# kaiwenShen/Do-You-Really-Need-to-Pay-2-20-Hedge-Fund-Strategy-Replication-via-Machine-Learning

Hardware: AMD Instinct MI355X
Metric: seq/sec/node MTSS-WGAN-GP train (24x32 windows) at 1/2/4/8 GPUs; W-dist parity (higher is better)
Workload: dtype fp32; 1 GPU; global_batch=262144, batch_per_gpu=262144, seq_len=24, features=32, parallelism=dp1

## Files before the change

do-you-really-need-to-pay-2-20-hedge-fund-strategy-replication-via-machine-learning_amd/csrc/lstmf_grad.hip:

```cpp
#include "lstmf_dev.h"

#include <stdexcept>
#include <type_traits>

namespace hfrep {

constexpr int WF_R = 16, WF_LA = 272, WF_LD = 400;
template <int KX>
struct WFGeo {
  static constexpr int KR = KX + FH + 1;
  static constexpr int NI = (KR + 15) / 16;
  static_assert(NI <= 16 && 16 * 16 <= WF_LA, "wgrad i tiles");
  static constexpr int NX4 = WF_R * KX / 4, NH4 = WF_R * FH / 4, ND4 = WF_R * FG / 4;
  static constexpr int JX = (NX4 + 511) / 512, JH = (NH4 + 511) / 512, JD = (ND4 + 511) / 512;
};

template <int KX, int XR = KX>
__global__ void __launch_bounds__(512)
lstmf_wgrad_kernel(const float* __restrict__ X, const float* __restrict__ Hs, const float* __restrict__ D,
                   const float* __restrict__ Xd, const float* __restrict__ Hds, const float* __restrict__ Dd,
                   float* __restrict__ slab, int M, int Tn, int rows_per_wg) {
  using WG = WFGeo<KX>;
  constexpr int NI = WG::NI, KR = WG::KR;
  __shared__ __attribute__((aligned(16))) float As[2][WF_R * WF_LA];
  __shared__ __attribute__((aligned(16))) float Ds[2][WF_R * WF_LD];
  __shared__ __attribute__((aligned(16))) float trash4[4];
  const int tid = threadIdx.x, lane = tid & 63;
  const int w = __builtin_amdgcn_readfirstlane(tid >> 6);
  const int g = lane >> 4, c16 = lane & 15;
  const int mb = blockIdx.x * rows_per_wg, me = min(M, mb + rows_per_wg);
  for (int i = tid; i < 2 * WF_R * WF_LA; i += 512) (&As[0][0])[i] = 0.f;

  f32x4 acc[NI][3], accx[2];
#pragma unroll
  for (int it = 0; it < NI; ++it)
#pragma unroll
    for (int jj = 0; jj < 3; ++jj) acc[it][jj] = f32x4{0.f, 0.f, 0.f, 0.f};
  accx[0] = accx[1] = f32x4{0.f, 0.f, 0.f, 0.f};
  const int ie0 = min(2 * w, 15), ie1 = min(2 * w + 1, 15);

  f32x4 vx[WG::JX], vh[WG::JH], vd[WG::JD];
  for (int seg = 0; seg < (Xd ? 2 : 1); ++seg) {
    const float* Xs = seg ? Xd : X;
    const float* Hq = seg ? Hds : Hs;
    const float* Dq = seg ? Dd : D;
    const int hb = mb > 0 ? mb - 1 : 0, nr = me > mb ? me - mb : 0;
    const rsrc_t rx = make_rsrc(Xs + (size_t)mb * XR, nr * XR * 4);
    const rsrc_t rh = make_rsrc(Hq + (size_t)hb * FH, (nr ? me - hb : 0) * FH * 4);
    const rsrc_t rd = make_rsrc(Dq + (size_t)mb * FG, nr * FG * 4);
    auto load = [&](int m0) {
#pragma unroll
      for (int j = 0; j < WG::JX; ++j) {
        const int e = tid + 512 * j, r = e / (KX / 4), c = e - r * (KX / 4);
        const bool ok = e < WG::NX4 && m0 + r < me;
        vx[j] = ldx4<XR>(rx, ok ? ((m0 - mb + r) * XR + 4 * c) * 4 : kOOB, 0, 4 * c);
      }
#pragma unroll
      for (int j = 0; j < WG::JH; ++j) {
        const int e = tid + 512 * j, r = e / (FH / 4), c = e - r * (FH / 4);
        const int m = m0 + r;
        const bool ok = e < WG::NH4 && m < me && (m % Tn) != 0;
        vh[j] = __builtin_bit_cast(f32x4, __builtin_amdgcn_raw_buffer_load_b128(rh, ok ? ((m - 1 - hb) * FH + 4 * c) * 4 : kOOB, 0, 0));
      }
#pragma unroll
      for (int j = 0; j < WG::JD; ++j) {
        const int e = tid + 512 * j, r = e / (FG / 4), c = e - r * (FG / 4);
        const bool ok = e < WG::ND4 && m0 + r < me;
        vd[j] = __builtin_bit_cast(f32x4, __builtin_amdgcn_raw_buffer_load_b128(rd, ok ? ((m0 - mb + r) * FG + 4 * c) * 4 : kOOB, 0, 0));
      }
    };
    auto to_lds = [&](int buf) {
#pragma unroll
      for (int j = 0; j < WG::JX; ++j) {
        const int e = tid + 512 * j, r = e / (KX / 4), c = e - r * (KX / 4);
        *reinterpret_cast<f32x4*>(e < WG::NX4 ? &As[buf][r * WF_LA + 4 * c] : trash4) = vx[j];
      }
#pragma unroll
      for (int j = 0; j < WG::JH; ++j) {
        const int e = tid + 512 * j, r = e / (FH / 4), c = e - r * (FH / 4);
        *reinterpret_cast<f32x4*>(e < WG::NH4 ? &As[buf][r * WF_LA + KX + 4 * c] : trash4) = vh[j];
      }
#pragma unroll
      for (int j = 0; j < WG::JD; ++j) {
        const int e = tid + 512 * j, r = e / (FG / 4), c = e - r * (FG / 4);
        *reinterpret_cast<f32x4*>(e < WG::ND4 ? &Ds[buf][r * WF_LD + 4 * c] : trash4) = vd[j];
      }
    };
    __syncthreads();
    if (tid < 2 * WF_R) As[tid >> 4][(tid & 15) * WF_LA + KR - 1] = seg ? 0.f : 1.f;
    if (mb < me) {
      load(mb);
      to_lds(0);
    }
    __syncthreads();
    int buf = 0;
    for (int m0 = mb; m0 < me; m0 += WF_R) {
      const bool more = m0 + WF_R < me;
      if (more) load(m0 + WF_R);
      const float* A_ = As[buf];
      const float* D_ = Ds[buf];
#pragma unroll
      for (int ks = 0; ks < 4; ++ks) {
        const float* ar = A_ + (4 * ks + g) * WF_LA + c16;
        const float* dr = D_ + (4 * ks + g) * WF_LD + c16;
        float a[NI], b[3];
#pragma unroll
        for (int it = 0; it < NI; ++it) a[it] = ar[16 * it];
#pragma unroll
        for (int jj = 0; jj < 3; ++jj) b[jj] = dr[16 * (3 * w + jj)];
        const float bx = dr[16 * 24], ax0 = ar[16 * ie0], ax1 = ar[16 * ie1];
#pragma unroll
        for (int it = 0; it < NI; ++it)
#pragma unroll
          for (int jj = 0; jj < 3; ++jj) acc[it][jj] = mma4(a[it], b[jj], acc[it][jj]);
        accx[0] = mma4(ax0, bx, accx[0]);
        accx[1] = mma4(ax1, bx, accx[1]);
      }
      if (more) to_lds(buf ^ 1);
      buf ^= 1;
      __syncthreads();
    }
  }
  float* out = slab + (size_t)blockIdx.x * KR * FG;
#pragma unroll
  for (int it = 0; it < NI; ++it)
#pragma unroll
    for (int jj = 0; jj < 3; ++jj)
#pragma unroll
      for (int r = 0; r < 4; ++r) {
        const int i = 16 * it + 4 * g + r;
        if (i < KR) out[(size_t)i * FG + 16 * (3 * w + jj) + c16] = acc[it][jj][r];
      }
#pragma unroll
  for (int e = 0; e < 2; ++e) {
    const int it = 2 * w + e;
#pragma unroll
    for (int r = 0; r < 4; ++r) {
      const int i = 16 * it + 4 * g + r;
      if (it < NI && i < KR) out[(size_t)i * FG + 16 * 24 + c16] = accx[e][r];
    }
  }
}

constexpr int WS_CA = 208, WS_CD = 208;
constexpr int ws_row_bytes(int cols, bool cf) {
  const int dw = (cols + 1) / 2;
  return 4 * (cf ? dw + ((8 - dw % 64) + 64) % 64 : (dw + 3) / 4 * 4);
}
template <int CA, int CD>
struct WImg {
  static constexpr bool CF = 2 * 3 * 32 * (ws_row_bytes(CA, true) + ws_row_bytes(CD, true)) <= 160 * 1024;
  static constexpr int ROWA = ws_row_bytes(CA, CF), ROWD = ws_row_bytes(CD, CF);
  static constexpr int PLA = 32 * ROWA, PLD = 32 * ROWD;
  static constexpr int IMGD = 3 * PLA;
  static constexpr int BUF = 3 * PLA + 3 * PLD;
  static_assert(2 * BUF <= 160 * 1024, "wgrad split LDS");
};

template <int KX>
struct WSGeo {
  static constexpr int KR = KX + FH + 1;
  static constexpr int NI = (KR + 15) / 16;
  static constexpr int NI0 = (NI + 1) / 2;
  static constexpr int JX = (32 * KX / 4 + 511) / 512, JH = (32 * FH / 4 + 511) / 512;
  static constexpr int JD = (32 * 52 + 511) / 512;
  static_assert(KX % 4 == 0 && 16 * NI <= WS_CA, "wgrad split: K");
  using Img = WImg<16 * NI, WS_CD>;
};

__device__ __forceinline__ int tr_lane_off(int lane, int rowb) {
  return (4 * (lane >> 4) + ((lane & 15) >> 2)) * rowb + 8 * (lane & 3);
}
template <int ROWB>
__device__ __forceinline__ bf16x8 tr_frag(const lds_char* img, int lane_off, int c0) {
  const s16x4 a = __builtin_amdgcn_ds_read_tr16_b64_v4i16((lds_s16x4*)(img + lane_off + c0 * 2));
  const s16x4 b = __builtin_amdgcn_ds_read_tr16_b64_v4i16((lds_s16x4*)(img + lane_off + 16 * ROWB + c0 * 2));
  return bf16x8{a[0], a[1], a[2], a[3], b[0], b[1], b[2], b[3]};
}

template <int NP>
__device__ __forceinline__ void wg_block(int Z, int& z, int& jp) {
  if (Z % 8 == 0) {
    const unsigned slot = blockIdx.x >> 3;
    jp = slot % NP;
    z = (slot / NP) * 8 + (blockIdx.x & 7);
  } else {
    jp = blockIdx.x % NP;
    z = blockIdx.x / NP;
  }
}
template <int BYTES>
__device__ __forceinline__ void wg_zero_lds(lds_char* wsm, int tid) {
  for (int i = tid; i < BYTES / 16; i += 512) reinterpret_cast<__attribute__((address_space(3))) u32x4_t*>(wsm)[i] = u32x4_t{0, 0, 0, 0};
}
template <class GI, int KR>
__device__ __forceinline__ void wg_bias_col(lds_char* wsm, int t, int seg) {
  if (t < 64) {
    const int buf = t >> 5, r = t & 31;
    *reinterpret_cast<__attribute__((address_space(3))) uint16_t*>(wsm + buf * GI::BUF + r * GI::ROWA + (KR - 1) * 2) =
        seg ? 0 : 0x3f80;
  }
}
struct WgRsrc {
  rsrc_t x, h, d;
};
template <int XR>
__device__ __forceinline__ WgRsrc wg_rsrc(const float* X, const float* H, const float* D, int mb, int nr, int jbase, int ncol) {
  return {make_rsrc(X + (size_t)mb * XR, nr * XR * 4), make_rsrc(H + ((ptrdiff_t)mb - 1) * FH, (nr ? nr + 1 : 0) * FH * 4),
          make_rsrc(D + (size_t)mb * FG + jbase, nr ? ((nr - 1) * FG + ncol) * 4 : 0)};
}
__device__ __forceinline__ int wg_tm0(int mb, int r, int Tn) { return (mb + r) % Tn; }
__device__ __forceinline__ void wg_tm_next(int& tm, int step32, int Tn) {
  tm += step32;
  if (tm >= Tn) tm -= Tn;
}
struct WgSlot {
  int r, c4;
  bool ok;
};
template <int PER>
__device__ __forceinline__ WgSlot wg_slot(int e) {
  const int r = e / PER;
  return {r, e - r * PER, e < 32 * PER};
}
template <int PER>
__device__ __forceinline__ WgSlot wg_slot(int e, int nc4) {
  WgSlot s = wg_slot<PER>(e);
  s.ok = s.ok && s.c4 < nc4;
  return s;
}
template <int RS>
__device__ __forceinline__ int wg_goff(const WgSlot& s) { return s.ok ? (s.r * RS + 4 * s.c4) * 4 : kOOB; }
template <int ROWB, int IMG>
__device__ __forceinline__ int wg_loff(const WgSlot& s) { return s.ok ? s.r * ROWB + IMG + 8 * s.c4 : -1; }
template <class GI>
__device__ __forceinline__ void wg_tr_bases(int lane, int (&tro_a)[2], int (&tro_d)[2]) {
#pragma unroll
  for (int b = 0; b < 2; ++b) {
    tro_a[b] = tr_lane_off(lane, GI::ROWA) + b * GI::BUF;
    tro_d[b] = tr_lane_off(lane, GI::ROWD) + b * GI::BUF + GI::IMGD;
    asm volatile("" : "+v"(tro_a[b]), "+v"(tro_d[b]));
  }
}
template <int KR>
__device__ __forceinline__ void wg_store_tile(float* out, const f32x4& acc, int it, int jt, int jbase, int ncol, int lane) {
  const int g = lane >> 4, col = 16 * jt + (lane & 15);
#pragma unroll
  for (int r = 0; r < 4; ++r) {
    const int i = 16 * it + 4 * g + r;
    if (i < KR && col < ncol) out[(size_t)i * FG + jbase + col] = acc[r];
  }
}

template <class GI, int NIV, int NJV, int NA, int NB>
__device__ __forceinline__ void ws_chunk(f32x4 (&acc)[NA][NB], const lds_char* A_, const lds_char* D_, int tro_a,
                                         int tro_d, int i0, int j0) {
  bf16x8 bfr[NJV][3];
#pragma unroll
  for (int jj = 0; jj < NJV; ++jj)
#pragma unroll
    for (int q = 0; q < 3; ++q) bfr[jj][q] = tr_frag<GI::ROWD>(D_ + q * GI::PLD, tro_d, 16 * (j0 + jj));
#pragma unroll
  for (int ii = 0; ii < NIV; ++ii) {
    __builtin_amdgcn_sched_barrier(0);
    bf16x8 a3[3];
#pragma unroll
    for (int q = 0; q < 3; ++q) a3[q] = tr_frag<GI::ROWA>(A_ + q * GI::PLA, tro_a, 16 * (i0 + ii));
#pragma unroll
    for (int j2 = 0; j2 < NJV; j2 += 2) {
      f32x4 t[2];
#pragma unroll
      for (int jj = j2; jj < j2 + 2 && jj < NJV; ++jj) t[jj - j2] = mma_split6(a3, bfr[jj], f32x4{0.f, 0.f, 0.f, 0.f});
#pragma unroll
      for (int jj = j2; jj < j2 + 2 && jj < NJV; ++jj) acc[ii][jj] += t[jj - j2];
    }
  }
}

template <int KX, int XR = KX>
__global__ void __launch_bounds__(512, 1)
lstmf_wgrad_split_kernel(const float* __restrict__ X, const float* __restrict__ Hs, const float* __restrict__ D,
                         const float* __restrict__ Xd, const float* __restrict__ Hds, const float* __restrict__ Dd,
                         float* __restrict__ slab, int M, int Tn, int rows_per_z, int Z) {
  constexpr int XRB = 4 * XR, HRB = 4 * FH, DRB = 4 * FG;
  using G = WSGeo<KX>;
  using GI = typename G::Img;
  constexpr int NI = G::NI, NI0 = G::NI0, JX = G::JX, JH = G::JH, JD = G::JD;
  extern __shared__ __attribute__((aligned(16))) char wsm_[];
  lds_char* wsm = (lds_char*)wsm_;
  const int tid = threadIdx.x, lane = tid & 63;
  const int w = __builtin_amdgcn_readfirstlane(tid >> 6);
  int z, jh;
  wg_block<2>(Z, z, jh);
  const int mb = z * rows_per_z, me = min(M, mb + rows_per_z);
  const int jbase = WS_CD * jh, nd4 = jh ? 48 : 52;

  const int ig = w >> 2, jg = ig ? 3 - (w & 3) : (w & 3);
  const int i0 = ig ? NI0 : 0, ni = ig ? NI - NI0 : NI0;
  const int j0 = jg == 0 ? 0 : 1 + 3 * jg, nj = jg == 0 ? 4 : 3;

  wg_zero_lds<2 * GI::BUF>(wsm, tid);
  __syncthreads();

  f32x4 acc[NI0][4];
#pragma unroll
  for (int a = 0; a < NI0; ++a)
#pragma unroll
    for (int b = 0; b < 4; ++b) acc[a][b] = f32x4{0.f, 0.f, 0.f, 0.f};

  const int tro_a = tr_lane_off(lane, GI::ROWA);
  int tro_d = tr_lane_off(lane, GI::ROWD) + GI::IMGD;
  asm volatile("" : "+v"(tro_d));

  int gx[JX], lx[JX], gh[JH], lh[JH], rhr[JH], gd[JD], ld_[JD], rd_[JD];
#pragma unroll
  for (int j = 0; j < JX; ++j) {
    const int e = tid + 512 * j, r = e / (KX / 4), c4 = e - r * (KX / 4);
    const bool ok = e < 32 * KX / 4;
    gx[j] = ok ? (r * XR + 4 * c4) * 4 : kOOB;
    lx[j] = ok ? r * GI::ROWA + 8 * c4 : -1;
  }
#pragma unroll
  for (int j = 0; j < JH; ++j) {
    const int e = tid + 512 * j, r = e / (FH / 4), c4 = e - r * (FH / 4);
    const bool ok = e < 32 * FH / 4;
    gh[j] = ok ? (r * FH + 4 * c4) * 4 : kOOB;
    lh[j] = ok ? r * GI::ROWA + 2 * KX + 8 * c4 : -1;
    rhr[j] = ok ? r : 0;
  }
#pragma unroll
  for (int j = 0; j < JD; ++j) {
    const int e = tid + 512 * j, r = e / 52, c4 = e - r * 52;
    const bool ok = e < 32 * 52 && c4 < nd4;
    gd[j] = ok ? (r * FG + jbase + 4 * c4) * 4 : kOOB;
    ld_[j] = ok ? GI::IMGD + r * GI::ROWD + 8 * c4 : -1;
    rd_[j] = ok ? r : 0;
  }
  const int step32 = 32 % Tn;

  f32x4 vx[JX], vh[JH], vd[JD];
  for (int seg = 0; seg < (Xd ? 2 : 1); ++seg) {
    const char* Xs = reinterpret_cast<const char*>(seg ? Xd : X);
    const char* Hq = reinterpret_cast<const char*>(seg ? Hds : Hs);
    const char* Dq = reinterpret_cast<const char*>(seg ? Dd : D);
    const int nr = me > mb ? me - mb : 0;
    const rsrc_t rx = make_rsrc(Xs + (size_t)mb * XRB, nr * XRB);
    const rsrc_t rh = make_rsrc(Hq + ((ptrdiff_t)mb - 1) * HRB, (nr ? nr + 1 : 0) * HRB);
    const rsrc_t rd = make_rsrc(Dq + (size_t)mb * DRB, nr * DRB);
    int tm[JH];
#pragma unroll
    for (int j = 0; j < JH; ++j) tm[j] = wg_tm0(mb, rhr[j], Tn);
    auto load = [&](int m0) {
      const int lim = me - m0;
#pragma unroll
      for (int j = 0; j < JX; ++j) {
        vx[j] = ldx4<XR>(rx, (gx[j] >> 2) / XR < lim ? gx[j] : kOOB, (m0 - mb) * XRB, (gx[j] >> 2) % XR);
      }
#pragma unroll
      for (int j = 0; j < JH; ++j) {
        const int vo = rhr[j] < lim && tm[j] != 0 ? gh[j] : kOOB;
        vh[j] = ld4s(rh, vo, (m0 - mb) * HRB);
      }
#pragma unroll
      for (int j = 0; j < JD; ++j) {
        const int vo = rd_[j] < lim ? gd[j] : kOOB;
        vd[j] = ld4s(rd, vo, (m0 - mb) * DRB);
      }
#pragma unroll
      for (int j = 0; j < JH; ++j) {
        wg_tm_next(tm[j], step32, Tn);
      }
    };
    auto put = [&](lds_char* base, int lo, const f32x4& v) {
      if (lo >= 0) {
        uint32_t p[3][2];
        split3(v, p);
        const int pl = lo < GI::IMGD ? GI::PLA : GI::PLD;
#pragma unroll
        for (int q = 0; q < 3; ++q)
          *reinterpret_cast<__attribute__((address_space(3))) u32x2_t*>(base + lo + q * pl) = u32x2_t{p[q][0], p[q][1]};
      }
    };
    auto stage = [&](int buf) {
      lds_char* base = wsm + buf * GI::BUF;
#pragma unroll
      for (int j = 0; j < JX; ++j) put(base, lx[j], vx[j]);
#pragma unroll
      for (int j = 0; j < JH; ++j) put(base, lh[j], vh[j]);
#pragma unroll
      for (int j = 0; j < JD; ++j) put(base, ld_[j], vd[j]);
    };
    wg_bias_col<GI, G::KR>(wsm, tid, seg);
    const int nch = nr > 0 ? (nr + 31) / 32 : 0;
    if (nch > 0) {
      load(mb);
      stage(0);
    }
    __syncthreads();
    for (int c = 0; c < nch; ++c) {
      const bool more = c + 1 < nch;
      if (more) load(mb + 32 * (c + 1));
      const lds_char* A_ = wsm + (c & 1) * GI::BUF;
      const lds_char* D_ = A_;
      switch (ni * 8 + nj) {
        case NI0 * 8 + 4: ws_chunk<GI, NI0, 4>(acc, A_, D_, tro_a, tro_d, i0, j0); break;
        case NI0 * 8 + 3: ws_chunk<GI, NI0, 3>(acc, A_, D_, tro_a, tro_d, i0, j0); break;
        case (NI - NI0) * 8 + 4: ws_chunk<GI, NI - NI0, 4>(acc, A_, D_, tro_a, tro_d, i0, j0); break;
        default: ws_chunk<GI, NI - NI0, 3>(acc, A_, D_, tro_a, tro_d, i0, j0); break;
      }
      if (more) stage((c + 1) & 1);
      __syncthreads();
    }
    __syncthreads();
  }
  float* out = slab + (size_t)z * G::KR * FG;
  const int g = lane >> 4, c16 = lane & 15;
#pragma unroll
  for (int ii = 0; ii < NI0; ++ii)
#pragma unroll
    for (int jj = 0; jj < 4; ++jj)
      if (ii < ni && jj < nj) {
        const int col = jbase + 16 * (j0 + jj) + c16;
#pragma unroll
        for (int r = 0; r < 4; ++r) {
          const int i = 16 * (i0 + ii) + 4 * g + r;
          if (i < G::KR && col < FG) out[(size_t)i * FG + col] = acc[ii][jj][r];
        }
      }
}

constexpr int WQ_CD = 100, WQ_NJ = 7, WQ_W = 8;
template <int KX>
struct WQGeo {
  static constexpr int KR = KX + FH + 1;
  static constexpr int NI = (KR + 15) / 16;
  static constexpr int NIG = (NI + 3) / 4;
  static constexpr int MAXT = NIG * 4;
  static constexpr int JX = (32 * KX / 4 + 511) / 512, JH = (32 * FH / 4 + 511) / 512;
  static constexpr int JD = (32 * WQ_CD / 4 + 511) / 512;
  static constexpr int NS = JX + JH + JD;
  static_assert(KX % 4 == 0 && 16 * NI <= WS_CA && NI <= 16, "wgrad q4: K");
  static constexpr int ig(int w) { return w < 4 ? w : 3 - (w & 3); }
  static constexpr int i0(int g) { return g == 0 ? 0 : NIG + (g - 1) * ((NI - NIG) / 3) + ((g - 1) < (NI - NIG) % 3 ? g - 1 : (NI - NIG) % 3); }
  static constexpr int ni(int g) { return i0(g + 1 > 3 ? 3 : g + 1) - i0(g) + (g == 3 ? NI - i0(3) : 0); }
  static constexpr int j0(int w) { return w < 4 ? 0 : 4; }
  static constexpr int nj(int w) { return w < 4 ? 4 : 3; }
  using Img = WImg<16 * NI, 16 * WQ_NJ>;
};

template <int KX>
__global__ void __launch_bounds__(512, 1)
lstmf_wgrad_q4_kernel(const float* __restrict__ X, const float* __restrict__ Hs, const float* __restrict__ D,
                      const float* __restrict__ Xd, const float* __restrict__ Hds, const float* __restrict__ Dd,
                      float* __restrict__ slab, int M, int Tn, int rows_per_z, int Z) {
  constexpr int XRB = 4 * KX, HRB = 4 * FH, DRB = 4 * FG;
  using G = WQGeo<KX>;
  using GI = typename G::Img;
  constexpr int JX = G::JX, JH = G::JH, NS = G::NS, MAXT = G::MAXT;
  extern __shared__ __attribute__((aligned(16))) char wsm_[];
  lds_char* wsm = (lds_char*)wsm_;
  const int tid = threadIdx.x, lane = tid & 63;
  const int w = __builtin_amdgcn_readfirstlane(tid >> 6);
  int z, jq;
  wg_block<4>(Z, z, jq);
  const int mb = z * rows_per_z, me = min(M, mb + rows_per_z);
  const int jbase = WQ_CD * jq;

  wg_zero_lds<2 * GI::BUF>(wsm, tid);
  __syncthreads();

  f32x4 acc[MAXT];
#pragma unroll
  for (int a = 0; a < MAXT; ++a) acc[a] = f32x4{0.f, 0.f, 0.f, 0.f};

  int tro_a[2], tro_d[2];
#pragma unroll
  for (int b = 0; b < 2; ++b) {
    tro_a[b] = tr_lane_off(lane, GI::ROWA) + b * GI::BUF;
    tro_d[b] = tr_lane_off(lane, GI::ROWD) + b * GI::BUF + GI::IMGD;
    asm volatile("" : "+v"(tro_a[b]), "+v"(tro_d[b]));
  }
  const int step32 = 32 % Tn;

  auto slot_rc = [&](int s, int& r, int& c4, bool& ok) {
    WgSlot sl;
    if (s < JX) sl = wg_slot<KX / 4>(tid + 512 * s);
    else if (s < JX + JH) sl = wg_slot<FH / 4>(tid + 512 * (s - JX));
    else sl = wg_slot<WQ_CD / 4>(tid + 512 * (s - JX - JH));
    r = sl.r; c4 = sl.c4; ok = sl.ok;
    if (!ok) r = c4 = 0;
  };

  f32x4 v[NS];
  for (int seg = 0; seg < (Xd ? 2 : 1); ++seg) {
    const char* Xs = reinterpret_cast<const char*>(seg ? Xd : X);
    const char* Hq = reinterpret_cast<const char*>(seg ? Hds : Hs);
    const char* Dq = reinterpret_cast<const char*>(seg ? Dd : D);
    const int nr = me > mb ? me - mb : 0;
    const rsrc_t rx = make_rsrc(Xs + (size_t)mb * XRB, nr * XRB);
    const rsrc_t rh = make_rsrc(Hq + ((ptrdiff_t)mb - 1) * HRB, (nr ? nr + 1 : 0) * HRB);
    const rsrc_t rd = make_rsrc(Dq + (size_t)mb * DRB + jbase * 4, nr ? (nr - 1) * DRB + WQ_CD * 4 : 0);
    int tm[JH];
#pragma unroll
    for (int j = 0; j < JH; ++j) {
      int r, c4;
      bool ok;
      slot_rc(JX + j, r, c4, ok);
      tm[j] = wg_tm0(mb, r, Tn);
    }
    auto load_slot = [&](int s, int m0) {
      int r, c4;
      bool ok;
      slot_rc(s, r, c4, ok);
      ok = ok && r < me - m0;
      if (s < JX) {
        v[s] = ld4s(rx, ok ? (r * KX + 4 * c4) * 4 : kOOB, (m0 - mb) * XRB);
      } else if (s < JX + JH) {
        int& tmj = tm[s - JX];
        v[s] = ld4s(rh, ok && tmj != 0 ? (r * FH + 4 * c4) * 4 : kOOB, (m0 - mb) * HRB);
        tmj += step32;
        if (tmj >= Tn) tmj -= Tn;
      } else {
        v[s] = ld4s(rd, ok ? (r * FG + 4 * c4) * 4 : kOOB, (m0 - mb) * DRB);
      }
    };
    auto stage = [&](lds_char* base, int s) {
      int r, c4;
      bool ok;
      slot_rc(s, r, c4, ok);
      if (!ok) return;
      int lo, pl;
      if (s < JX) { lo = r * GI::ROWA + 8 * c4; pl = GI::PLA; }
      else if (s < JX + JH) { lo = r * GI::ROWA + 2 * KX + 8 * c4; pl = GI::PLA; }
      else { lo = GI::IMGD + r * GI::ROWD + 8 * c4; pl = GI::PLD; }
      uint32_t p[3][2];
      split3(v[s], p);
#pragma unroll
      for (int q = 0; q < 3; ++q)
        *reinterpret_cast<__attribute__((address_space(3))) u32x2_t*>(base + lo + q * pl) = u32x2_t{p[q][0], p[q][1]};
    };
    using I0 = std::integral_constant<int, 0>;
    using I1 = std::integral_constant<int, 1>;
    wg_bias_col<GI, G::KR>(wsm, tid, seg);
    const int nch = nr > 0 ? (nr + 31) / 32 : 0;
#pragma unroll
    for (int s = 0; s < NS; ++s) load_slot(s, mb);
#pragma unroll
    for (int s = 0; s < NS; ++s) stage(wsm, s);
#pragma unroll
    for (int s = 0; s < NS; ++s) load_slot(s, mb + 32);
    __syncthreads();
    auto chunk = [&](auto S_, int c) {
      constexpr int S = decltype(S_)::value;
      const lds_char* A_ = wsm;
      const lds_char* D_ = wsm;
      lds_char* nxt = wsm + (S ^ 1) * GI::BUF;
      auto body = [&](auto WK) {
        constexpr int W = decltype(WK)::value;
        constexpr int IG = G::ig(W), I0 = G::i0(IG), NIW = G::ni(IG), J0 = G::j0(W), NJW = G::nj(W);
        constexpr int NJH = (NJW + 1) / 2;
        constexpr int SPI = (NS + NJH * NIW - 1) / (NJH * NIW);
        auto jpair = [&](auto JH_) {
          constexpr int jh = decltype(JH_)::value;
          bf16x8 bfr[2][3];
#pragma unroll
          for (int jj = 0; jj < 2; ++jj)
            if (2 * jh + jj < NJW) {
#pragma unroll
              for (int q = 0; q < 3; ++q) bfr[jj][q] = tr_frag<GI::ROWD>(D_ + q * GI::PLD, tro_d[S], 16 * (J0 + 2 * jh + jj));
            }
          constexpr bool PF = KX <= 36;
          bf16x8 af[2][3];
#pragma unroll
          for (int q = 0; q < 3; ++q) af[0][q] = tr_frag<GI::ROWA>(A_ + q * GI::PLA, tro_a[S], 16 * I0);
#pragma unroll
          for (int ii = 0; ii < NIW; ++ii) {
            __builtin_amdgcn_sched_barrier(0);
            if (PF && ii + 1 < NIW) {
#pragma unroll
              for (int q = 0; q < 3; ++q) af[(ii + 1) & 1][q] = tr_frag<GI::ROWA>(A_ + q * GI::PLA, tro_a[S], 16 * (I0 + ii + 1));
            } else if (!PF && ii > 0) {
#pragma unroll
              for (int q = 0; q < 3; ++q) af[ii & 1][q] = tr_frag<GI::ROWA>(A_ + q * GI::PLA, tro_a[S], 16 * (I0 + ii));
            }
            const bf16x8(&a3)[3] = af[ii & 1];
#pragma unroll
            for (int jj = 0; jj < 2; ++jj) {
              if (2 * jh + jj >= NJW) continue;
              acc[ii * 4 + 2 * jh + jj] += mma_split6(a3, bfr[jj], f32x4{0.f, 0.f, 0.f, 0.f});
            }
            const int it = jh * NIW + ii;
#pragma unroll
            for (int s = it * SPI; s < (it + 1) * SPI && s < NS; ++s) {
              stage(nxt, s);
              load_slot(s, mb + 32 * (c + 2));
            }
          }
        };
        jpair(std::integral_constant<int, 0>{});
        if constexpr (NJH > 1) jpair(std::integral_constant<int, 1>{});
      };
      switch (w) {
        case 0: body(std::integral_constant<int, 0>{}); break;
        case 1: body(std::integral_constant<int, 1>{}); break;
        case 2: body(std::integral_constant<int, 2>{}); break;
        case 3: body(std::integral_constant<int, 3>{}); break;
        case 4: body(std::integral_constant<int, 4>{}); break;
        case 5: body(std::integral_constant<int, 5>{}); break;
        case 6: body(std::integral_constant<int, 6>{}); break;
        default: body(std::integral_constant<int, 7>{}); break;
      }
      __syncthreads();
    };
    int c = 0;
    for (; c + 1 < nch; c += 2) {
      chunk(I0{}, c);
      chunk(I1{}, c + 1);
    }
    if (c < nch) chunk(I0{}, c);
    __syncthreads();
  }
  float* out = slab + (size_t)z * G::KR * FG;
  const int g = lane >> 4, c16 = lane & 15;
  const int igw = G::ig(w), i0w = G::i0(igw), niw = G::ni(igw), j0w = G::j0(w), njw = G::nj(w);
#pragma unroll
  for (int ii = 0; ii < G::NIG; ++ii)
#pragma unroll
    for (int jj = 0; jj < 4; ++jj) {
      const int col = 16 * (j0w + jj) + c16;
#pragma unroll
      for (int r = 0; r < 4; ++r) {
        const int i = 16 * (i0w + ii) + 4 * g + r;
        if (ii < niw && jj < njw && i < G::KR && col < WQ_CD)
          out[(size_t)i * FG + jbase + col] = acc[ii * 4 + jj][r];
      }
    }
}

#ifndef HFREP_WGRAD_ROLES_APF
#define HFREP_WGRAD_ROLES_APF 1
#endif
#ifndef HFREP_WGRAD_ROLES_PRIO
#define HFREP_WGRAD_ROLES_PRIO 0
#endif
template <int KX>
struct WRGeo {
  static constexpr bool QUAD = KX > 36;
  static constexpr int NP = QUAD ? 4 : 2;
  static constexpr int CDP = QUAD ? WQ_CD : WS_CD;
  static constexpr int NJ = (CDP + 15) / 16;
  static constexpr int KR = KX + FH + 1;
  static constexpr int NI = (KR + 15) / 16;
  static constexpr int NT = NI * NJ;
  static constexpr int ts(int w) { return w * (NT / 4) + (w < NT % 4 ? w : NT % 4); }
  static constexpr int MAXT = (NT + 3) / 4;
  static constexpr int ND4 = CDP / 4;
  static constexpr int JX = (32 * KX / 4 + 255) / 256, JH = (32 * FH / 4 + 255) / 256, JD = (32 * ND4 + 255) / 256;
  static constexpr int NS = JX + JH + JD;
  static_assert(KX % 4 == 0 && CDP % 4 == 0 && 16 * NI <= WS_CA && MAXT * 4 <= 120, "wgrad roles: K");
  using Img = WImg<16 * NI, 16 * NJ>;
};

template <int KX>
__global__ void __launch_bounds__(512, 1)
lstmf_wgrad_roles_kernel(const float* __restrict__ X, const float* __restrict__ Hs, const float* __restrict__ D,
                         const float* __restrict__ Xd, const float* __restrict__ Hds, const float* __restrict__ Dd,
                         float* __restrict__ slab, int M, int Tn, int rows_per_z, int Z) {
  using G = WRGeo<KX>;
  using GI = typename G::Img;
  constexpr int NI = G::NI, NP = G::NP, JX = G::JX, JH = G::JH, NS = G::NS;
  constexpr int XRB = 4 * KX, HRB = 4 * FH, DRB = 4 * FG;
  extern __shared__ __attribute__((aligned(16))) char wsm_[];
  lds_char* wsm = (lds_char*)wsm_;
  const int tid = threadIdx.x, lane = tid & 63;
  const int w = __builtin_amdgcn_readfirstlane(tid >> 6);
  int z, jp;
  wg_block<NP>(Z, z, jp);
  const int mb = z * rows_per_z, me = min(M, mb + rows_per_z);
  const int jbase = G::CDP * jp, ncol = min(G::CDP, FG - jbase);
  const int nr = me > mb ? me - mb : 0, nch = (nr + 31) / 32;
  const int nseg = Xd ? 2 : 1;

  wg_zero_lds<2 * GI::BUF>(wsm, tid);
  __syncthreads();

  using I0 = std::integral_constant<int, 0>;
  using I1 = std::integral_constant<int, 1>;
  if (w < 4) {
    auto role = [&](auto WK) {
      constexpr int W = decltype(WK)::value;
      constexpr int TS = G::ts(W), TE = G::ts(W + 1), JA = TS / NI, NJW = (TE - 1) / NI - JA + 1;
      f32x4 acc[TE - TS];
#pragma unroll
      for (int a = 0; a < TE - TS; ++a) acc[a] = f32x4{0.f, 0.f, 0.f, 0.f};
      int tro_a[2], tro_d[2];
      wg_tr_bases<GI>(lane, tro_a, tro_d);
      auto chunk = [&](auto S_) {
        constexpr int S = decltype(S_)::value;
        bf16x8 bfr[NJW][3];
#pragma unroll
        for (int jj = 0; jj < NJW; ++jj)
#pragma unroll
          for (int q = 0; q < 3; ++q) bfr[jj][q] = tr_frag<GI::ROWD>(wsm + q * GI::PLD, tro_d[S], 16 * (JA + jj));
        constexpr int PF = HFREP_WGRAD_ROLES_APF;
        bf16x8 af[PF + 1][3];
#pragma unroll
        for (int i = 0; i < PF; ++i)
#pragma unroll
          for (int q = 0; q < 3; ++q) af[i][q] = tr_frag<GI::ROWA>(wsm + q * GI::PLA, tro_a[S], 16 * i);
        f32x4 t[2];
        int pend = -1, par = 0;
#pragma unroll
        for (int ii = 0; ii < NI; ++ii) {
          __builtin_amdgcn_sched_barrier(0);
          if (ii + PF < NI) {
#pragma unroll
            for (int q = 0; q < 3; ++q) af[(ii + PF) % (PF + 1)][q] = tr_frag<GI::ROWA>(wsm + q * GI::PLA, tro_a[S], 16 * (ii + PF));
          }
          __builtin_amdgcn_sched_barrier(0);
          const bf16x8(&a3)[3] = af[ii % (PF + 1)];
#pragma unroll
          for (int jj = 0; jj < NJW; ++jj) {
            const int L = (JA + jj) * NI + ii;
            if (L < TS || L >= TE) continue;
            t[par] = mma_split6(a3, bfr[jj], f32x4{0.f, 0.f, 0.f, 0.f});
            __builtin_amdgcn_sched_barrier(0);
            if (pend >= 0) acc[pend] += t[par ^ 1];
            pend = L - TS;
            par ^= 1;
            __builtin_amdgcn_sched_barrier(0);
          }
        }
        acc[pend] += t[par ^ 1];
      };
#if HFREP_WGRAD_ROLES_PRIO
      __builtin_amdgcn_s_setprio(1);
#endif
      for (int seg = 0; seg < nseg; ++seg) {
        lds_barrier();
        int c = 0;
        for (; c + 1 < nch; c += 2) {
          chunk(I0{});
          lds_barrier();
          chunk(I1{});
          lds_barrier();
        }
        if (c < nch) {
          chunk(I0{});
          lds_barrier();
        }
      }
      float* out = slab + (size_t)z * G::KR * FG;
#pragma unroll
      for (int n = 0; n < TE - TS; ++n) wg_store_tile<G::KR>(out, acc[n], (TS + n) % NI, (TS + n) / NI, jbase, ncol, lane);
    };
    switch (w) {
      case 0: role(std::integral_constant<int, 0>{}); break;
      case 1: role(std::integral_constant<int, 1>{}); break;
      case 2: role(std::integral_constant<int, 2>{}); break;
      default: role(std::integral_constant<int, 3>{}); break;
    }
  } else {
    const int st = tid - 256;
    int gv[NS], lo[NS], rr[NS];
#pragma unroll
    for (int s = 0; s < NS; ++s) {
      WgSlot sl;
      if (s < JX) {
        sl = wg_slot<KX / 4>(st + 256 * s);
        gv[s] = wg_goff<KX>(sl);
        lo[s] = wg_loff<GI::ROWA, 0>(sl);
      } else if (s < JX + JH) {
        sl = wg_slot<FH / 4>(((st + 64) & 255) + 256 * (s - JX));
        gv[s] = wg_goff<FH>(sl);
        lo[s] = wg_loff<GI::ROWA, 2 * KX>(sl);
      } else {
        sl = wg_slot<G::ND4>(((st + 128) & 255) + 256 * (s - JX - JH), ncol / 4);
        gv[s] = wg_goff<FG>(sl);
        lo[s] = wg_loff<GI::ROWD, GI::IMGD>(sl);
      }
      rr[s] = sl.ok ? sl.r : 0;
    }
    const int step32 = 32 % Tn;
    f32x4 v[2][NS];
    for (int seg = 0; seg < nseg; ++seg) {
      const WgRsrc rs = wg_rsrc<KX>(seg ? Xd : X, seg ? Hds : Hs, seg ? Dd : D, mb, nr, jbase, ncol);
      int tm[JH];
#pragma unroll
      for (int j = 0; j < JH; ++j) tm[j] = wg_tm0(mb, rr[JX + j], Tn);
      auto load = [&](auto Q_, int m0) {
        constexpr int Q = decltype(Q_)::value;
        const int lim = me - m0;
#pragma unroll
        for (int s = 0; s < NS; ++s) {
          const bool in = rr[s] < lim;
          if (s < JX) {
            v[Q][s] = ld4s(rs.x, in ? gv[s] : kOOB, (m0 - mb) * XRB);
          } else if (s < JX + JH) {
            int& tmj = tm[s - JX];
            v[Q][s] = ld4s(rs.h, in && tmj != 0 ? gv[s] : kOOB, (m0 - mb) * HRB);
            wg_tm_next(tmj, step32, Tn);
          } else {
            v[Q][s] = ld4s(rs.d, in ? gv[s] : kOOB, (m0 - mb) * DRB);
          }
        }
      };
      auto stage = [&](auto Q_, int buf) {
        constexpr int Q = decltype(Q_)::value;
        lds_char* base = wsm + buf * GI::BUF;
#pragma unroll
        for (int s = 0; s < NS; ++s) {
          if (lo[s] >= 0) split3_store(v[Q][s], base + lo[s], s < JX + JH ? GI::PLA : GI::PLD);
        }
      };
      wg_bias_col<GI, G::KR>(wsm, st, seg);
      load(I0{}, mb);
      stage(I0{}, 0);
      load(I1{}, mb + 32);
      lds_barrier();
      int c = 0;
      for (; c + 1 < nch; c += 2) {
        load(I0{}, mb + 32 * (c + 2));
        stage(I1{}, 1);
        lds_barrier();
        load(I1{}, mb + 32 * (c + 3));
        stage(I0{}, 0);
        lds_barrier();
      }
      if (c < nch) {
        load(I0{}, mb + 32 * (c + 2));
        stage(I1{}, 1);
        lds_barrier();
      }
    }
  }
}

constexpr int DS4_RS = 432;
constexpr int DS4_PL = 16 * DS4_RS * 2;
constexpr int DS4_BUF = 3 * DS4_PL;
constexpr int DS4_SLOTS = (16 * 100 + 255) / 256;
constexpr int DS4_K0 = DS_KS - DS4_SLOTS;
constexpr int DS4_NS = 2;

template <int NT2>
__global__ void __launch_bounds__(256, 1)
lstmf_dgrad_s4_kernel(const float* __restrict__ D, const float* __restrict__ W, float* __restrict__ X, int M, int KO) {
  constexpr int DRB = 4 * FG;
  extern __shared__ __attribute__((aligned(16))) char dsm_[];
  lds_char* dsm = (lds_char*)dsm_;
  const int tid = threadIdx.x, lane = tid & 63;
  const int w = __builtin_amdgcn_readfirstlane(tid >> 6);
  const int g = lane >> 4, c16 = lane & 15;
  const int nch = (M + 15) / 16;
  bf16x8 bw[2][DS_KS][3];
#pragma unroll
  for (int e = 0; e < 2; ++e) {
    const int col = 16 * (2 * w + e) + c16;
#pragma unroll
    for (int ks = 0; ks < DS_KS; ++ks) {
      const int k0 = 32 * ks + 8 * g;
      f32x4 v0 = f32x4{0.f, 0.f, 0.f, 0.f}, v1 = v0;
      if (w < NT2 && col < KO && k0 < FG) {
        v0 = *reinterpret_cast<const f32x4*>(W + (size_t)col * FG + k0);
        v1 = *reinterpret_cast<const f32x4*>(W + (size_t)col * FG + k0 + 4);
      }
      uint32_t p0[3][2], p1[3][2];
      split3(v0, p0);
      split3(v1, p1);
#pragma unroll
      for (int q = 0; q < 3; ++q) {
        bw[e][ks][q] = __builtin_bit_cast(bf16x8, make_uint4(p0[q][0], p0[q][1], p1[q][0], p1[q][1]));
        if (e == 1) asm volatile("" : "+a"(bw[e][ks][q]));
      }
    }
  }
  f32x4 v[DS4_NS][DS4_SLOTS];
  auto load = [&](auto S_, int c) {
    constexpr int S = decltype(S_)::value;
    const int r0 = c * 16, nr = c < nch ? min(16, M - r0) : 0;
    const rsrc_t rd = make_rsrc(reinterpret_cast<const char*>(D) + (nr ? (size_t)r0 * DRB : 0), nr * DRB);
#pragma unroll
    for (int j = 0; j < DS4_SLOTS; ++j) {
      const int e = tid + 256 * j, r = e / 100, c4 = e - 100 * r;
      v[S][j] = ld4(rd, e < 1600 ? (r * FG + 4 * c4) * 4 : kOOB);
    }
  };
  auto stage = [&](auto S_, lds_char* buf, int j) {
    constexpr int S = decltype(S_)::value;
    const int e = tid + 256 * j, r = e / 100, c4 = e - 100 * r;
    if (e >= 1600) return;
    const int lo = (r * DS4_RS + 4 * c4) * 2;
    split3_store(v[S][j], buf + lo, DS4_PL);
  };
  for (int i = tid; i < 2 * 3 * 16 * 2; i += 256) {
    const int h = i & 1, b = i / 96, q = (i / 32) % 3, r = (i / 2) % 16;
    *reinterpret_cast<__attribute__((address_space(3))) u32x4_t*>(dsm + b * DS4_BUF + q * DS4_PL +
                                                                  (r * DS4_RS + FG + 8 * h) * 2) = u32x4_t{0, 0, 0, 0};
  }
  using I0 = std::integral_constant<int, 0>;
  using I1 = std::integral_constant<int, 1>;
  const int cs = gridDim.x;
  load(I0{}, blockIdx.x);
#pragma unroll
  for (int j = 0; j < DS4_SLOTS; ++j) stage(I0{}, dsm, j);
  load(I1{}, blockIdx.x + cs);
  __syncthreads();
  const int ao = (c16 * DS4_RS + 8 * g) * 2;
  auto chunk = [&](auto S_, int cc, int P) {
    constexpr int S = decltype(S_)::value, SN = (S + 1) % DS4_NS;
    load(S_, cc + DS4_NS * cs);
    const lds_char* A_ = dsm + P * DS4_BUF;
    lds_char* nxt = dsm + (P ^ 1) * DS4_BUF;
    f32x4 acc[2] = {f32x4{0.f, 0.f, 0.f, 0.f}, f32x4{0.f, 0.f, 0.f, 0.f}};
    bf16x8 af[2][3];
#pragma unroll
    for (int q = 0; q < 3; ++q) af[0][q] = *reinterpret_cast<const __attribute__((address_space(3))) bf16x8*>(A_ + q * DS4_PL + ao);
#pragma unroll
    for (int ks = 0; ks < DS_KS; ++ks) {
      __builtin_amdgcn_sched_barrier(0);
      if (ks + 1 < DS_KS) {
#pragma unroll
        for (int q = 0; q < 3; ++q)
          af[(ks + 1) & 1][q] = *reinterpret_cast<const __attribute__((address_space(3))) bf16x8*>(A_ + q * DS4_PL + ao + 64 * (ks + 1));
      }
      const bf16x8(&a)[3] = af[ks & 1];
#pragma unroll
      for (int e = 0; e < 2; ++e) acc[e] = mma_split6(a, bw[e][ks], acc[e]);
      if (ks >= DS4_K0) {
        stage(std::integral_constant<int, SN>{}, nxt, ks - DS4_K0);
#pragma unroll
        for (int i = 0; i < 12; ++i) {
          __builtin_amdgcn_sched_group_barrier(0x008, 1, 0);
          __builtin_amdgcn_sched_group_barrier(0x002, 2, 0);
        }
      }
    }
    const int nr = min(16, M - 16 * cc);
    const rsrc_t rx = make_rsrc(X + (size_t)16 * cc * KO, nr * KO * 4);
#pragma unroll
    for (int e = 0; e < 2; ++e) {
      const int col = 16 * (2 * w + e) + c16;
      const bool ok = w < NT2 && col < KO;
#pragma unroll
      for (int i = 0; i < 4; ++i) st1(acc[e][i], rx, ok ? ((4 * g + i) * KO + col) * 4 : kOOB, 0);
    }
    __syncthreads();
  };
  int c = blockIdx.x;
  for (; c + cs < nch; c += 2 * cs) {
    chunk(I0{}, c, 0);
    chunk(I1{}, c + cs, 1);
  }
  if (c < nch) chunk(I0{}, c, 0);
}

constexpr int DG_KS = 25;
template <int NT>
__global__ void __launch_bounds__(256, 1)
lstmf_dgrad_kernel(const float* __restrict__ D, const float* __restrict__ W, float* __restrict__ X, int M, int KO,
                   int rows_per_wg) {
  __shared__ __attribute__((aligned(16))) f32x4 part[2][4][NT][64];
  const int tid = threadIdx.x, lane = tid & 63;
  const int w = __builtin_amdgcn_readfirstlane(tid >> 6);
  const int g = lane >> 4, c16 = lane & 15;
  const int mb = blockIdx.x * rows_per_wg, nrows = min(M, mb + rows_per_wg) - mb;
  if (nrows <= 0) return;
  const int kb = 100 * w;

  float bw[NT][DG_KS];
#pragma unroll
  for (int n = 0; n < NT; ++n) {
    const int col = 16 * n + c16;
#pragma unroll
    for (int s = 0; s < DG_KS; ++s) {
      const int k = s < 24 ? kb + 16 * (s >> 2) + 4 * g + (s & 3) : kb + 96 + g;
      bw[n][s] = col < KO ? W[col * FG + k] : 0.f;
    }
  }
  const rsrc_t rd = make_rsrc(D + (size_t)mb * FG, nrows * FG * 4);
  const rsrc_t rx = make_rsrc(X + (size_t)mb * KO, nrows * KO * 4);
  const int nch = (nrows + 15) / 16;

  f32x4 a0[6], a1[6], acc0[NT], acc1[NT];
  float s0 = 0.f, s1 = 0.f;
  auto load = [&](f32x4 (&a)[6], float& a_s, int r0) {
    const int vo = ((r0 + c16) * FG + kb + 4 * g) * 4;
#pragma unroll
    for (int q = 0; q < 6; ++q) a[q] = __builtin_bit_cast(f32x4, __builtin_amdgcn_raw_buffer_load_b128(rd, vo + 64 * q, 0, 0));
    a_s = ld1(rd, vo + (96 - 3 * g) * 4, 0);
  };
  auto mm = [&](f32x4 (&acc)[NT], const f32x4 (&a)[6], int q0, int q1) {
#pragma unroll
    for (int q = q0; q < q1; ++q)
#pragma unroll
      for (int j = 0; j < 4; ++j)
#pragma unroll
        for (int n = 0; n < NT; ++n) acc[n] = mma4(a[q][j], bw[n][4 * q + j], acc[n]);
  };
  auto put = [&](const f32x4 (&acc)[NT], int slot) {
#pragma unroll
    for (int n = 0; n < NT; ++n) part[slot][w][n][lane] = acc[n];
  };
  auto reduce = [&](int slot, int r0, bool on) {
#pragma unroll
    for (int e = 0; e < (NT * 64 + 255) / 256; ++e) {
      const int idx = tid + 256 * e, ok = on && idx < NT * 64, ix = idx < NT * 64 ? idx : 0;
      const int n = ix >> 6, ln = ix & 63, col = 16 * n + (ln & 15), row = r0 + 4 * (ln >> 4);
      const f32x4 v = ((part[slot][0][n][ln] + part[slot][1][n][ln]) + part[slot][2][n][ln]) + part[slot][3][n][ln];
#pragma unroll
      for (int i = 0; i < 4; ++i) st1(v[i], rx, ok && col < KO ? ((row + i) * KO + col) * 4 : kOOB, 0);
    }
  };
  auto chunk = [&](f32x4 (&cur)[NT], const f32x4 (&prev)[NT], const f32x4 (&a)[6], float a_s, f32x4 (&an)[6],
                   float& an_s, int c) {
    reduce(c & 1, 16 * (c - 2), c >= 2);
    load(an, an_s, 16 * (c + 1));
    __builtin_amdgcn_sched_barrier(0);
#pragma unroll
    for (int n = 0; n < NT; ++n) cur[n] = f32x4{0.f, 0.f, 0.f, 0.f};
    mm(cur, a, 0, 2);
    if (c >= 1) put(prev, (c - 1) & 1);
    mm(cur, a, 2, 6);
#pragma unroll
    for (int n = 0; n < NT; ++n) cur[n] = mma4(a_s, bw[n][24], cur[n]);
    __syncthreads();
  };

  load(a0, s0, 0);
  int c = 0;
  for (; c + 2 <= nch; c += 2) {
    chunk(acc0, acc1, a0, s0, a1, s1, c);
    chunk(acc1, acc0, a1, s1, a0, s0, c + 1);
  }
  if (c < nch) chunk(acc0, acc1, a0, s0, a1, s1, c++);
  if (c & 1)
    put(acc0, (c - 1) & 1);
  else
    put(acc1, (c - 1) & 1);
  reduce(c & 1, 16 * (c - 2), c >= 2);
  __syncthreads();
  reduce((c - 1) & 1, 16 * (c - 1), true);
}

bool lstmf_wgrad_supported(int K, int H, int N) { return H == FH && N == FG && (K == 32 || K == 35 || K == 36 || K == 100); }

static int wgradf_pick(int impl, int K) {
  int v = impl >= 1 && impl <= 4 ? impl : (fp32_exact() ? 1 : 0);
  if (K == 35 && v == 3) v = 2;
  const bool roles = K == 32 || K == 100;
  if (v == 0) v = roles ? 4 : 0;
  if (v == 4 && !roles) v = 0;
  return v ? v : (K <= 36 ? 2 : 3);
}
struct WgradPart {
  int np, z, rows, zcap;
};
static WgradPart wgradf_part(int v, int K, int M) {
  const int np = v == 1 ? 1 : v == 3 || (v == 4 && K == 100) ? 4 : 2;
  if (M <= 0) return {np, 0, 0, 0};
  const int ch = v == 1 ? WF_R : 32;
  const int chunks = (M + ch - 1) / ch, wgs = device_cu_count() / np;
  const int z0 = chunks < wgs ? chunks : wgs;
  const int rows = ((M + z0 - 1) / z0 + ch - 1) / ch * ch;
  return {np, (M + rows - 1) / rows, rows, z0};
}
size_t lstmf_wgrad_workspace_floats(int M, int K, int impl) {
  return (size_t)wgradf_part(wgradf_pick(impl, K), K, M).zcap * ((K == 35 ? 36 : K) + FH + 1) * FG;
}

bool launch_lstmf_wgrad(const float* X, const float* Hs, const float* D, const float* Xd, const float* Hds, const float* Dd,
                        float* gW, float* gU, float* gb, int M, int K, int Tn, float* ws, hipStream_t s, int impl) {
  if (!lstmf_wgrad_supported(K, FH, FG) || M <= 0) return false;
  const int v = wgradf_pick(impl, K);
  const WgradPart p = wgradf_part(v, K, M);
  auto go = [&](auto k, size_t sm) {
    allow_lds(reinterpret_cast<const void*>(k));
    hipLaunchKernelGGL(k, dim3(p.np * p.z), dim3(512), sm, s, X, Hs, D, Xd, Hds, Dd, ws, M, Tn, p.rows, p.z);
  };
  auto exact = [&](auto k) { hipLaunchKernelGGL(k, dim3(p.z), dim3(512), 0, s, X, Hs, D, Xd, Hds, Dd, ws, M, Tn, p.rows); };
  switch (v * 128 + K) {
    case 1 * 128 + 32: exact(lstmf_wgrad_kernel<32>); break;
    case 1 * 128 + 35: exact(lstmf_wgrad_kernel<36, 35>); break;
    case 1 * 128 + 36: exact(lstmf_wgrad_kernel<36>); break;
    case 1 * 128 + 100: exact(lstmf_wgrad_kernel<100>); break;
    case 2 * 128 + 32: go(lstmf_wgrad_split_kernel<32>, 2 * WSGeo<32>::Img::BUF); break;
    case 2 * 128 + 35: go(lstmf_wgrad_split_kernel<36, 35>, 2 * WSGeo<36>::Img::BUF); break;
    case 2 * 128 + 36: go(lstmf_wgrad_split_kernel<36>, 2 * WSGeo<36>::Img::BUF); break;
    case 2 * 128 + 100: go(lstmf_wgrad_split_kernel<100>, 2 * WSGeo<100>::Img::BUF); break;
    case 3 * 128 + 32: go(lstmf_wgrad_q4_kernel<32>, 2 * WQGeo<32>::Img::BUF); break;
    case 3 * 128 + 36: go(lstmf_wgrad_q4_kernel<36>, 2 * WQGeo<36>::Img::BUF); break;
    case 3 * 128 + 100: go(lstmf_wgrad_q4_kernel<100>, 2 * WQGeo<100>::Img::BUF); break;
    case 4 * 128 + 32: go(lstmf_wgrad_roles_kernel<32>, 2 * WRGeo<32>::Img::BUF); break;
    case 4 * 128 + 100: go(lstmf_wgrad_roles_kernel<100>, 2 * WRGeo<100>::Img::BUF); break;
    default: throw std::runtime_error("lstmf_wgrad: no kernel for this impl / K");
  }
  launch_lstm_wgrad2_reduce(ws, gW, gU, gb, p.z, K, FH, FG, s, K == 35 ? 36 : K);
  return true;
}

bool lstmf_dgrad_supported(int N, int KO) { return N == FG && KO >= 1 && KO <= 16 * FNT; }

bool launch_lstmf_dgrad(const float* D, const float* W, float* X, int M, int N, int KO, hipStream_t s, int impl) {
  if (!lstmf_dgrad_supported(N, KO) || M <= 0) return false;
  const int dv = impl == 1 || impl == 3 ? impl : (fp32_exact() ? 1 : 0);
  if (dv == 3 || (dv == 0 && KO > 64)) {
    const int chunks = (M + 15) / 16, cus = device_cu_count();
    const int grid = chunks < cus ? chunks : cus;
    auto go = [&](auto k) {
      allow_lds(reinterpret_cast<const void*>(k));
      hipLaunchKernelGGL(k, dim3(grid), dim3(256), (size_t)2 * DS4_BUF, s, D, W, X, M, KO);
    };
    switch ((KO + 31) / 32) {
      case 1: go(lstmf_dgrad_s4_kernel<1>); break;
      case 2: go(lstmf_dgrad_s4_kernel<2>); break;
      case 3: go(lstmf_dgrad_s4_kernel<3>); break;
      default: go(lstmf_dgrad_s4_kernel<4>); break;
    }
    return true;
  }
  const int chunks = (M + 15) / 16, cus = device_cu_count() * (KO <= 48 ? 2 : 1);
  int grid = chunks < cus ? chunks : cus;
  const int min_grid = (int)(((long long)M * FG * 4 + (1ll << 31) - 1) / (1ll << 31));
  if (grid < min_grid) grid = min_grid;
  const int rpw = (chunks + grid - 1) / grid * 16;
  const int z = (M + rpw - 1) / rpw;
  switch ((KO + 15) / 16) {
    case 1: hipLaunchKernelGGL(lstmf_dgrad_kernel<1>, dim3(z), dim3(256), 0, s, D, W, X, M, KO, rpw); break;
    case 2: hipLaunchKernelGGL(lstmf_dgrad_kernel<2>, dim3(z), dim3(256), 0, s, D, W, X, M, KO, rpw); break;
    case 3: hipLaunchKernelGGL(lstmf_dgrad_kernel<3>, dim3(z), dim3(256), 0, s, D, W, X, M, KO, rpw); break;
    case 4: hipLaunchKernelGGL(lstmf_dgrad_kernel<4>, dim3(z), dim3(256), 0, s, D, W, X, M, KO, rpw); break;
    case 5: hipLaunchKernelGGL(lstmf_dgrad_kernel<5>, dim3(z), dim3(256), 0, s, D, W, X, M, KO, rpw); break;
    case 6: hipLaunchKernelGGL(lstmf_dgrad_kernel<6>, dim3(z), dim3(256), 0, s, D, W, X, M, KO, rpw); break;
    default: hipLaunchKernelGGL(lstmf_dgrad_kernel<7>, dim3(z), dim3(256), 0, s, D, W, X, M, KO, rpw); break;
  }
  return true;
}

}
```

Baseline: 1.541 million seq/s.

## Add warp-specialized dgrad kernel with producer waves staging D into LDS

Adds a 512-thread dgrad kernel in which seven waves compute split-bf16 MFMA products while an eighth producer wave, plus a few slots shared by the compute waves, streams D chunks from global memory into double-buffered LDS with a prefetch depth of two. The default path for KO > 64 now uses this kernel instead of the s4 kernel, with the old kernel still reachable as impl 3. The goal is to hide global load latency behind matrix math. The cost is more waves per CU, more register pressure from the producer buffers, and a barrier on every chunk.

```diff
diff --git a/do-you-really-need-to-pay-2-20-hedge-fund-strategy-replication-via-machine-learning_amd/csrc/lstmf_grad.hip b/do-you-really-need-to-pay-2-20-hedge-fund-strategy-replication-via-machine-learning_amd/csrc/lstmf_grad.hip
--- a/do-you-really-need-to-pay-2-20-hedge-fund-strategy-replication-via-machine-learning_amd/csrc/lstmf_grad.hip
+++ b/do-you-really-need-to-pay-2-20-hedge-fund-strategy-replication-via-machine-learning_amd/csrc/lstmf_grad.hip
@@ -955,6 +955,164 @@
   if (c < nch) chunk(I0{}, c, 0);
 }
 
+#ifndef HFREP_DGRAD_ROLES_SHARE
+#define HFREP_DGRAD_ROLES_SHARE 2
+#endif
+#ifndef HFREP_DGRAD_ROLES_DEPTH
+#define HFREP_DGRAD_ROLES_DEPTH 2
+#endif
+constexpr int DR_SH = HFREP_DGRAD_ROLES_SHARE, DR_D = HFREP_DGRAD_ROLES_DEPTH;
+constexpr int DR_SLOTS = 16 * (FG / 4) / 64;
+constexpr int DR_NS = DR_SLOTS - 7 * DR_SH;
+constexpr int DR_K0 = 2, DR_KST = 3;
+static_assert(DR_SH >= 0 && DR_SH <= 3 && (DR_D == 1 || DR_D == 2), "dgrad roles: share / depth");
+
+__global__ void __launch_bounds__(512, 1)
+lstmf_dgrad_roles_kernel(const float* __restrict__ D, const float* __restrict__ W, float* __restrict__ X, int M, int KO) {
+  constexpr int DRB = 4 * FG;
+  extern __shared__ __attribute__((aligned(16))) char drm_[];
+  lds_char* dsm = (lds_char*)drm_;
+  const int tid = threadIdx.x, lane = tid & 63;
+  const int w = __builtin_amdgcn_readfirstlane(tid >> 6);
+  const int nch = (M + 15) / 16, cs = gridDim.x, cb = blockIdx.x;
+  for (int i = tid; i < 2 * 3 * 16 * 2; i += 512) {
+    const int h = i & 1, b = i / 96, q = (i / 32) % 3, r = (i / 2) % 16;
+    *reinterpret_cast<__attribute__((address_space(3))) u32x4_t*>(dsm + b * DS4_BUF + q * DS4_PL +
+                                                                  (r * DS4_RS + FG + 8 * h) * 2) = u32x4_t{0, 0, 0, 0};
+  }
+  auto drsrc = [&](int c) {
+    const int r0 = c * 16, nr = c < nch ? min(16, M - r0) : 0;
+    return make_rsrc(reinterpret_cast<const char*>(D) + (nr ? (size_t)r0 * DRB : 0), nr * DRB);
+  };
+  auto slot_lo = [&](int s) {
+    const int e = lane + 64 * s, r = e / 100;
+    return (r * DS4_RS + 4 * (e - 100 * r)) * 2;
+  };
+  using I0 = std::integral_constant<int, 0>;
+  using I1 = std::integral_constant<int, 1>;
+  if (w < 7) {
+    const int g = lane >> 4, c16 = lane & 15, col = 16 * w + c16;
+    bf16x8 bw[DS_KS][3];
+    const rsrc_t rw = make_rsrc(W, KO * FG * 4);
+    int wrow = col * FG * 4;
+#pragma unroll
+    for (int ks = 0; ks < DS_KS; ++ks) {
+      if (ks) asm volatile("" : "+v"(wrow), "+v"(bw[ks - 1][0]), "+v"(bw[ks - 1][1]), "+v"(bw[ks - 1][2]));
+      const int k0 = 32 * ks + 8 * g, wo = col < KO && k0 < FG ? wrow + k0 * 4 : kOOB;
+      const f32x4 v0 = ld4(rw, wo), v1 = ld4(rw, wo == kOOB ? kOOB : wo + 16);
+      uint32_t p0[3][2], p1[3][2];
+      split3(v0, p0);
+      split3(v1, p1);
+#pragma unroll
+      for (int q = 0; q < 3; ++q) bw[ks][q] = __builtin_bit_cast(bf16x8, make_uint4(p0[q][0], p0[q][1], p1[q][0], p1[q][1]));
+    }
+    const int ao = (c16 * DS4_RS + 8 * g) * 2;
+    int xo[4];
+#pragma unroll
+    for (int i = 0; i < 4; ++i) {
+      xo[i] = col < KO ? ((4 * g + i) * KO + col) * 4 : kOOB;
+      asm volatile("" : "+v"(xo[i]));
+    }
+    constexpr int NX = DR_SH ? DR_SH : 1;
+    int xg[NX], xl[NX];
+    f32x4 vx[DR_D][NX];
+#pragma unroll
+    for (int i = 0; i < DR_SH; ++i) {
+      const int xs = DR_NS + DR_SH * w + i;
+      xg[i] = 16 * (lane + 64 * xs);
+      xl[i] = slot_lo(xs);
+    }
+#pragma unroll
+    for (int s = 0; s < DR_D; ++s) {
+      const rsrc_t rd = drsrc(cb + s * cs);
+#pragma unroll
+      for (int i = 0; i < DR_SH; ++i) vx[s][i] = ld4(rd, xg[i]);
+    }
+    {
+      const rsrc_t rd = drsrc(cb + DR_D * cs);
+#pragma unroll
+      for (int i = 0; i < DR_SH; ++i) {
+        split3_store(vx[0][i], dsm + xl[i], DS4_PL);
+        vx[0][i] = ld4(rd, xg[i]);
+      }
+    }
+    lds_barrier();
+    auto chunk = [&](auto P_, int cc) {
+      constexpr int P = decltype(P_)::value, Q = P ^ 1, S = Q % DR_D;
+      const lds_char* A_ = dsm + P * DS4_BUF + ao;
+      const rsrc_t rdn = drsrc(cc + (1 + DR_D) * cs);
+      f32x4 acc = f32x4{0.f, 0.f, 0.f, 0.f};
+      bf16x8 af[2][3];
+#pragma unroll
+      for (int q = 0; q < 3; ++q) af[0][q] = *reinterpret_cast<const __attribute__((address_space(3))) bf16x8*>(A_ + q * DS4_PL);
+#pragma unroll
+      for (int ks = 0; ks < DS_KS; ++ks) {
+        __builtin_amdgcn_sched_barrier(0);
+        if (ks + 1 < DS_KS) {
+#pragma unroll
+          for (int q = 0; q < 3; ++q)
+            af[(ks + 1) & 1][q] = *reinterpret_cast<const __attribute__((address_space(3))) bf16x8*>(A_ + q * DS4_PL + 64 * (ks + 1));
+        }
+        __builtin_amdgcn_sched_barrier(0);
+        acc = mma_split6(af[ks & 1], bw[ks], acc);
+#pragma unroll
+        for (int i = 0; i < DR_SH; ++i) {
+          if (ks == DR_K0 + DR_KST * i) {
+            split3_store(vx[S][i], dsm + Q * DS4_BUF + xl[i], DS4_PL);
+#pragma unroll
+            for (int n = 0; n < 6; ++n) {
+              __builtin_amdgcn_sched_group_barrier(0x008, 1, 0);
+              __builtin_amdgcn_sched_group_barrier(0x002, 4, 0);
+            }
+          }
+          if (ks == DR_K0 + DR_KST * i + 1) vx[S][i] = ld4(rdn, xg[i]);
+        }
+      }
+      const int nr = min(16, M - 16 * cc);
+      const rsrc_t rx = make_rsrc(X + (size_t)16 * cc * KO, nr * KO * 4);
+#pragma unroll
+      for (int i = 0; i < 4; ++i) st1(acc[i], rx, xo[i], 0);
+      lds_barrier();
+    };
+    for (int cc = cb;;) {
+      chunk(I0{}, cc);
+      if ((cc += cs) >= nch) break;
+      chunk(I1{}, cc);
+      if ((cc += cs) >= nch) break;
+    }
+  } else {
+    int lo[DR_NS];
+#pragma unroll
+    for (int j = 0; j < DR_NS; ++j) lo[j] = slot_lo(j);
+    f32x4 v[DR_D][DR_NS];
+    auto roll = [&](auto Q_, int c) {
+      constexpr int Q = decltype(Q_)::value, S = Q % DR_D;
+      const rsrc_t rd = drsrc(c);
+#pragma unroll
+      for (int j = 0; j < DR_NS; ++j) {
+        split3_store(v[S][j], dsm + Q * DS4_BUF + lo[j], DS4_PL);
+        v[S][j] = ld4(rd, 16 * (lane + 64 * j));
+      }
+    };
+#pragma unroll
+    for (int s = 0; s < DR_D; ++s) {
+      const rsrc_t rd = drsrc(cb + s * cs);
+#pragma unroll
+      for (int j = 0; j < DR_NS; ++j) v[s][j] = ld4(rd, 16 * (lane + 64 * j));
+    }
+    roll(I0{}, cb + DR_D * cs);
+    lds_barrier();
+    for (int cc = cb;;) {
+      roll(I1{}, cc + (1 + DR_D) * cs);
+      lds_barrier();
+      if ((cc += cs) >= nch) break;
+      roll(I0{}, cc + (1 + DR_D) * cs);
+      lds_barrier();
+      if ((cc += cs) >= nch) break;
+    }
+  }
+}
+
 constexpr int DG_KS = 25;
 template <int NT>
 __global__ void __launch_bounds__(256, 1)
@@ -1103,8 +1261,15 @@
 
 bool launch_lstmf_dgrad(const float* D, const float* W, float* X, int M, int N, int KO, hipStream_t s, int impl) {
   if (!lstmf_dgrad_supported(N, KO) || M <= 0) return false;
-  const int dv = impl == 1 || impl == 3 ? impl : (fp32_exact() ? 1 : 0);
-  if (dv == 3 || (dv == 0 && KO > 64)) {
+  const int dv = impl == 1 || impl == 3 || impl == 4 ? impl : (fp32_exact() ? 1 : 0);
+  if (dv == 4 || (dv == 0 && KO > 64)) {
+    const int chunks = (M + 15) / 16, cus = device_cu_count();
+    const int grid = chunks < cus ? chunks : cus;
+    allow_lds(reinterpret_cast<const void*>(lstmf_dgrad_roles_kernel));
+    hipLaunchKernelGGL(lstmf_dgrad_roles_kernel, dim3(grid), dim3(512), (size_t)2 * DS4_BUF, s, D, W, X, M, KO);
+    return true;
+  }
+  if (dv == 3) {
     const int chunks = (M + 15) / 16, cus = device_cu_count();
     const int grid = chunks < cus ? chunks : cus;
     auto go = [&](auto k) {
```

New measurement: 1.557 million seq/s (median of 6 runs). 1.1% higher.
